# jolibrain/joliGEN

Hardware: AMD Instinct MI355X
Metric: train images/sec at 256x256 (DDPM UNet step) (higher is better)
Workload: dtype bf16; 1 GPU; palette_model DDPM, efficient UNet unet_mha ngf64 mults[1,2,4,8] res_blocks[2,2,2,2] mid-attn 16x32, 256x256, batch 32/GPU, inpainting synthetic masks, AdamW+EMA, iter_size 1 (example_ddpm_noglasses2glasses.json + SURVEY Appendix C overrides); global_batch=32, per_gpu_batch=32, image_size=256, efficient=True, parallelism=dp1, n_ranks_seen=1

## Files before the change

joligen_amd/csrc/attention.hip:

```cpp
#include "common.h"

namespace {

constexpr int D = 32;
constexpr int BQ = 128;
constexpr int BK = 128;

__device__ __forceinline__ int fsw(int row) { return (-(row >> 2)) & 3; }
__device__ __forceinline__ int bsw(int row) { return (row >> 2) & 1; }

template <typename T, int MODE>
__device__ __forceinline__ void stage_load(const T* __restrict__ g, long ld, int tid, uint4* r) {
#pragma unroll
  for (int i = 0; i < 2; ++i) {
    const int pos = i * 256 + tid, row = pos >> 2, c = pos & 3;
    r[i] = *reinterpret_cast<const uint4*>(g + (long)row * ld + c * 8);
  }
}
template <int MODE>
__device__ __forceinline__ void stage_store(uint4* lds, int tid, const uint4* r) {
#pragma unroll
  for (int i = 0; i < 2; ++i) {
    const int pos = i * 256 + tid, row = pos >> 2, c = pos & 3;
    const int pc = MODE == 0 ? (c ^ fsw(row)) : ((((c >> 1) ^ bsw(row)) << 1) | (c & 1));
    lds[row * 4 + pc] = r[i];
  }
}
__device__ __forceinline__ uint4 frag_rows(const uint4* lds, int tile, int l15, int g) {
  const int row = tile * 16 + l15;
  return lds[row * 4 + (g ^ fsw(row))];
}
__device__ __forceinline__ uint4 frag_tr(const uint4* lds, int blk, int dt, int l15, int g) {
  const char* base = reinterpret_cast<const char*>(lds);
  uint32_t w[4];
#pragma unroll
  for (int h = 0; h < 2; ++h) {
    const int row = blk * 32 + h * 16 + g * 4 + (l15 >> 2);
    const int off = row * 64 + ((dt ^ bsw(row)) << 5) + (l15 & 3) * 8;
    const uint2 u = __builtin_bit_cast(uint2, __builtin_amdgcn_ds_read_tr16_b64_v4i16((lds_v4)(base + off)));
    w[2 * h] = u.x;
    w[2 * h + 1] = u.y;
  }
  return make_uint4(w[0], w[1], w[2], w[3]);
}
template <typename T> __device__ __forceinline__ uint4 pack_p(const f32x4& a, const f32x4& b) {
  float f[8] = {a[0], a[1], a[2], a[3], b[0], b[1], b[2], b[3]};
  return pack8<T>(f);
}

struct AttnP {
  const char* qkv; char* a; float* L;
  const char* da; const char* o; char* dqkv; float* Dq;
  int B, T, nh;
  float scale;
};

template <typename T>
__global__ __launch_bounds__(256) void attn_fwd_kernel(AttnP p) {
  __shared__ uint4 sK[2][BK * 4], sV[2][BK * 4];
  const int tid = threadIdx.x, lane = tid & 63, wave = tid >> 6;
  const int l15 = lane & 15, g = lane >> 4;
  const int bh = blockIdx.y, b = bh / p.nh, h = bh % p.nh;
  const int C3 = 3 * p.nh * D;
  const T* base = (const T*)p.qkv + (long)b * p.T * C3 + h * 3 * D;
  const int q0 = blockIdx.x * BQ + wave * 32;

  uint4 fq[2];
#pragma unroll
  for (int qt = 0; qt < 2; ++qt) fq[qt] = *reinterpret_cast<const uint4*>(base + (long)(q0 + qt * 16 + l15) * C3 + g * 8);

  const int nchunk = p.T / BK;
  uint4 rk[2], rv[2];

  float mrun[2] = {-1e30f, -1e30f}, lrun[2] = {0.f, 0.f};
  stage_load<T, 0>(base + D, C3, tid, rk);
  stage_store<0>(sK[0], tid, rk);
  __syncthreads();
  for (int c = 0; c < nchunk; ++c) {
    const int cur = c & 1;
    if (c + 1 < nchunk) stage_load<T, 0>(base + (long)(c + 1) * BK * C3 + D, C3, tid, rk);
#pragma unroll
    for (int kt = 0; kt < 8; ++kt) {
      const uint4 fk = frag_rows(sK[cur], kt, l15, g);
#pragma unroll
      for (int qt = 0; qt < 2; ++qt) {
        f32x4 s = Mfma<T>::run(fk, fq[qt], (f32x4){0.f, 0.f, 0.f, 0.f});
        float mx = fmaxf(fmaxf(s[0], s[1]), fmaxf(s[2], s[3])) * p.scale;
        const float mnew = fmaxf(mrun[qt], mx);
        float acc = lrun[qt] * __expf(mrun[qt] - mnew);
#pragma unroll
        for (int r = 0; r < 4; ++r) acc += __expf(s[r] * p.scale - mnew);
        mrun[qt] = mnew;
        lrun[qt] = acc;
      }
    }
    if (c + 1 < nchunk) stage_store<0>(sK[cur ^ 1], tid, rk);
    __syncthreads();
  }
  float Lq[2];
#pragma unroll
  for (int qt = 0; qt < 2; ++qt) {
    float m = mrun[qt];
    m = fmaxf(m, __shfl_xor(m, 16));
    m = fmaxf(m, __shfl_xor(m, 32));
    float l = lrun[qt] * __expf(mrun[qt] - m);
    l += __shfl_xor(l, 16);
    l += __shfl_xor(l, 32);
    Lq[qt] = m + __logf(l);
    if (g == 0) p.L[(long)bh * p.T + q0 + qt * 16 + l15] = Lq[qt];
  }

  f32x4 o[2][2];
#pragma unroll
  for (int qt = 0; qt < 2; ++qt)
#pragma unroll
    for (int dt = 0; dt < 2; ++dt) o[qt][dt] = (f32x4){0.f, 0.f, 0.f, 0.f};
  stage_load<T, 0>(base + D, C3, tid, rk);
  stage_load<T, 1>(base + 2 * D, C3, tid, rv);
  stage_store<0>(sK[0], tid, rk);
  stage_store<1>(sV[0], tid, rv);
  __syncthreads();
  for (int c = 0; c < nchunk; ++c) {
    const int cur = c & 1;
    if (c + 1 < nchunk) {
      stage_load<T, 0>(base + (long)(c + 1) * BK * C3 + D, C3, tid, rk);
      stage_load<T, 1>(base + (long)(c + 1) * BK * C3 + 2 * D, C3, tid, rv);
    }
#pragma unroll
    for (int kb = 0; kb < 4; ++kb) {
      const uint4 fk0 = frag_rows(sK[cur], 2 * kb, l15, g), fk1 = frag_rows(sK[cur], 2 * kb + 1, l15, g);
      const uint4 fv0 = frag_tr(sV[cur], kb, 0, l15, g), fv1 = frag_tr(sV[cur], kb, 1, l15, g);
#pragma unroll
      for (int qt = 0; qt < 2; ++qt) {
        f32x4 s0 = Mfma<T>::run(fk0, fq[qt], (f32x4){0.f, 0.f, 0.f, 0.f});
        f32x4 s1 = Mfma<T>::run(fk1, fq[qt], (f32x4){0.f, 0.f, 0.f, 0.f});
#pragma unroll
        for (int r = 0; r < 4; ++r) {
          s0[r] = __expf(s0[r] * p.scale - Lq[qt]);
          s1[r] = __expf(s1[r] * p.scale - Lq[qt]);
        }
        const uint4 fp = pack_p<T>(s0, s1);
        o[qt][0] = Mfma<T>::run(fp, fv0, o[qt][0]);
        o[qt][1] = Mfma<T>::run(fp, fv1, o[qt][1]);
      }
    }
    if (c + 1 < nchunk) {
      stage_store<0>(sK[cur ^ 1], tid, rk);
      stage_store<1>(sV[cur ^ 1], tid, rv);
    }
    __syncthreads();
  }
  T* ab = (T*)p.a + (long)b * p.T * (p.nh * D) + h * D;
#pragma unroll
  for (int qt = 0; qt < 2; ++qt)
#pragma unroll
    for (int dt = 0; dt < 2; ++dt)
#pragma unroll
      for (int r = 0; r < 4; ++r)
        ab[(long)(q0 + qt * 16 + g * 4 + r) * (p.nh * D) + dt * 16 + l15] = from_f32<T>(o[qt][dt][r]);
}

template <typename T>
__global__ __launch_bounds__(256) void attn_bwd_dq_kernel(AttnP p) {
  __shared__ uint4 sK[2][BK * 4], sKt[2][BK * 4], sV[2][BK * 4];
  const int tid = threadIdx.x, lane = tid & 63, wave = tid >> 6;
  const int l15 = lane & 15, g = lane >> 4;
  const int bh = blockIdx.y, b = bh / p.nh, h = bh % p.nh;
  const int C3 = 3 * p.nh * D, C1 = p.nh * D;
  const T* base = (const T*)p.qkv + (long)b * p.T * C3 + h * 3 * D;
  const T* dab = (const T*)p.da + (long)b * p.T * C1 + h * D;
  const T* ob = (const T*)p.o + (long)b * p.T * C1 + h * D;
  const int q0 = blockIdx.x * BQ + wave * 32;

  uint4 fq[2], fdo[2];
  float Lq[2], Dq[2];
#pragma unroll
  for (int qt = 0; qt < 2; ++qt) {
    const long q = q0 + qt * 16 + l15;
    fq[qt] = *reinterpret_cast<const uint4*>(base + q * C3 + g * 8);
    fdo[qt] = *reinterpret_cast<const uint4*>(dab + q * C1 + g * 8);
    const uint4 fo = *reinterpret_cast<const uint4*>(ob + q * C1 + g * 8);
    float a[8], c[8];
    unpack8<T>(fdo[qt], a);
    unpack8<T>(fo, c);
    float d = 0.f;
#pragma unroll
    for (int i = 0; i < 8; ++i) d += a[i] * c[i];
    d += __shfl_xor(d, 16);
    d += __shfl_xor(d, 32);
    Dq[qt] = d;
    Lq[qt] = p.L[(long)bh * p.T + q];
    if (g == 0) p.Dq[(long)bh * p.T + q] = d;
  }
  f32x4 dq[2][2];
#pragma unroll
  for (int qt = 0; qt < 2; ++qt)
#pragma unroll
    for (int dt = 0; dt < 2; ++dt) dq[qt][dt] = (f32x4){0.f, 0.f, 0.f, 0.f};

  const int nchunk = p.T / BK;
  uint4 rk[2], rv[2];
  stage_load<T, 0>(base + D, C3, tid, rk);
  stage_load<T, 0>(base + 2 * D, C3, tid, rv);
  stage_store<0>(sK[0], tid, rk);
  stage_store<1>(sKt[0], tid, rk);
  stage_store<0>(sV[0], tid, rv);
  __syncthreads();
  for (int c = 0; c < nchunk; ++c) {
    const int cur = c & 1;
    if (c + 1 < nchunk) {
      stage_load<T, 0>(base + (long)(c + 1) * BK * C3 + D, C3, tid, rk);
      stage_load<T, 0>(base + (long)(c + 1) * BK * C3 + 2 * D, C3, tid, rv);
    }
#pragma unroll
    for (int kb = 0; kb < 4; ++kb) {
      const uint4 fk0 = frag_rows(sK[cur], 2 * kb, l15, g), fk1 = frag_rows(sK[cur], 2 * kb + 1, l15, g);
      const uint4 fv0 = frag_rows(sV[cur], 2 * kb, l15, g), fv1 = frag_rows(sV[cur], 2 * kb + 1, l15, g);
      const uint4 fkt0 = frag_tr(sKt[cur], kb, 0, l15, g), fkt1 = frag_tr(sKt[cur], kb, 1, l15, g);
#pragma unroll
      for (int qt = 0; qt < 2; ++qt) {
        const f32x4 z = {0.f, 0.f, 0.f, 0.f};
        f32x4 s0 = Mfma<T>::run(fk0, fq[qt], z), s1 = Mfma<T>::run(fk1, fq[qt], z);
        f32x4 d0 = Mfma<T>::run(fv0, fdo[qt], z), d1 = Mfma<T>::run(fv1, fdo[qt], z);
#pragma unroll
        for (int r = 0; r < 4; ++r) {
          s0[r] = __expf(s0[r] * p.scale - Lq[qt]) * (d0[r] - Dq[qt]);
          s1[r] = __expf(s1[r] * p.scale - Lq[qt]) * (d1[r] - Dq[qt]);
        }
        const uint4 fds = pack_p<T>(s0, s1);
        dq[qt][0] = Mfma<T>::run(fds, fkt0, dq[qt][0]);
        dq[qt][1] = Mfma<T>::run(fds, fkt1, dq[qt][1]);
      }
    }
    if (c + 1 < nchunk) {
      stage_store<0>(sK[cur ^ 1], tid, rk);
      stage_store<1>(sKt[cur ^ 1], tid, rk);
      stage_store<0>(sV[cur ^ 1], tid, rv);
    }
    __syncthreads();
  }
  T* dqb = (T*)p.dqkv + (long)b * p.T * C3 + h * 3 * D;
#pragma unroll
  for (int qt = 0; qt < 2; ++qt)
#pragma unroll
    for (int dt = 0; dt < 2; ++dt)
#pragma unroll
      for (int r = 0; r < 4; ++r)
        dqb[(long)(q0 + qt * 16 + g * 4 + r) * C3 + dt * 16 + l15] = from_f32<T>(dq[qt][dt][r] * p.scale);
}

template <typename T>
__global__ __launch_bounds__(256) void attn_bwd_dkv_kernel(AttnP p) {
  __shared__ uint4 sQ[2][BK * 4], sQt[2][BK * 4], sO[2][BK * 4], sOt[2][BK * 4];
  __shared__ float sL[2][BK], sD[2][BK];
  const int tid = threadIdx.x, lane = tid & 63, wave = tid >> 6;
  const int l15 = lane & 15, g = lane >> 4;
  const int bh = blockIdx.y, b = bh / p.nh, h = bh % p.nh;
  const int C3 = 3 * p.nh * D, C1 = p.nh * D;
  const T* base = (const T*)p.qkv + (long)b * p.T * C3 + h * 3 * D;
  const T* dab = (const T*)p.da + (long)b * p.T * C1 + h * D;
  const int k0 = blockIdx.x * BQ + wave * 32;

  uint4 fk[2], fv[2];
#pragma unroll
  for (int kt = 0; kt < 2; ++kt) {
    fk[kt] = *reinterpret_cast<const uint4*>(base + (long)(k0 + kt * 16 + l15) * C3 + D + g * 8);
    fv[kt] = *reinterpret_cast<const uint4*>(base + (long)(k0 + kt * 16 + l15) * C3 + 2 * D + g * 8);
  }
  f32x4 dk[2][2], dv[2][2];
#pragma unroll
  for (int kt = 0; kt < 2; ++kt)
#pragma unroll
    for (int dt = 0; dt < 2; ++dt) dk[kt][dt] = dv[kt][dt] = (f32x4){0.f, 0.f, 0.f, 0.f};

  const int nchunk = p.T / BK;
  uint4 rq[2], ro[2];
  float rl = 0.f, rd = 0.f;
  auto load = [&](int c) {
    stage_load<T, 0>(base + (long)c * BK * C3, C3, tid, rq);
    stage_load<T, 0>(dab + (long)c * BK * C1, C1, tid, ro);
    if (tid < BK) {
      rl = p.L[(long)bh * p.T + c * BK + tid];
      rd = p.Dq[(long)bh * p.T + c * BK + tid];
    }
  };
  auto store = [&](int buf) {
    stage_store<0>(sQ[buf], tid, rq);
    stage_store<1>(sQt[buf], tid, rq);
    stage_store<0>(sO[buf], tid, ro);
    stage_store<1>(sOt[buf], tid, ro);
    if (tid < BK) {
      sL[buf][tid] = rl;
      sD[buf][tid] = rd;
    }
  };
  load(0);
  store(0);
  __syncthreads();
  for (int c = 0; c < nchunk; ++c) {
    const int cur = c & 1;
    if (c + 1 < nchunk) load(c + 1);
#pragma unroll
    for (int qb = 0; qb < 4; ++qb) {
      const uint4 fq0 = frag_rows(sQ[cur], 2 * qb, l15, g), fq1 = frag_rows(sQ[cur], 2 * qb + 1, l15, g);
      const uint4 fo0 = frag_rows(sO[cur], 2 * qb, l15, g), fo1 = frag_rows(sO[cur], 2 * qb + 1, l15, g);
      const uint4 fqt0 = frag_tr(sQt[cur], qb, 0, l15, g), fqt1 = frag_tr(sQt[cur], qb, 1, l15, g);
      const uint4 fot0 = frag_tr(sOt[cur], qb, 0, l15, g), fot1 = frag_tr(sOt[cur], qb, 1, l15, g);
      const float4 L0 = *reinterpret_cast<const float4*>(&sL[cur][qb * 32 + g * 4]);
      const float4 L1 = *reinterpret_cast<const float4*>(&sL[cur][qb * 32 + 16 + g * 4]);
      const float4 D0 = *reinterpret_cast<const float4*>(&sD[cur][qb * 32 + g * 4]);
      const float4 D1 = *reinterpret_cast<const float4*>(&sD[cur][qb * 32 + 16 + g * 4]);
      const float l0[4] = {L0.x, L0.y, L0.z, L0.w}, l1[4] = {L1.x, L1.y, L1.z, L1.w};
      const float e0[4] = {D0.x, D0.y, D0.z, D0.w}, e1[4] = {D1.x, D1.y, D1.z, D1.w};
#pragma unroll
      for (int kt = 0; kt < 2; ++kt) {
        const f32x4 z = {0.f, 0.f, 0.f, 0.f};
        f32x4 s0 = Mfma<T>::run(fq0, fk[kt], z), s1 = Mfma<T>::run(fq1, fk[kt], z);
        f32x4 d0 = Mfma<T>::run(fo0, fv[kt], z), d1 = Mfma<T>::run(fo1, fv[kt], z);
        f32x4 ds0, ds1;
#pragma unroll
        for (int r = 0; r < 4; ++r) {
          s0[r] = __expf(s0[r] * p.scale - l0[r]);
          s1[r] = __expf(s1[r] * p.scale - l1[r]);
          ds0[r] = s0[r] * (d0[r] - e0[r]);
          ds1[r] = s1[r] * (d1[r] - e1[r]);
        }
        const uint4 fp = pack_p<T>(s0, s1), fds = pack_p<T>(ds0, ds1);
        dv[kt][0] = Mfma<T>::run(fp, fot0, dv[kt][0]);
        dv[kt][1] = Mfma<T>::run(fp, fot1, dv[kt][1]);
        dk[kt][0] = Mfma<T>::run(fds, fqt0, dk[kt][0]);
        dk[kt][1] = Mfma<T>::run(fds, fqt1, dk[kt][1]);
      }
    }
    if (c + 1 < nchunk) store(cur ^ 1);
    __syncthreads();
  }
  T* dqb = (T*)p.dqkv + (long)b * p.T * C3 + h * 3 * D;
#pragma unroll
  for (int kt = 0; kt < 2; ++kt)
#pragma unroll
    for (int dt = 0; dt < 2; ++dt)
#pragma unroll
      for (int r = 0; r < 4; ++r) {
        const long row = (long)(k0 + kt * 16 + g * 4 + r) * C3 + dt * 16 + l15;
        dqb[row + D] = from_f32<T>(dk[kt][dt][r] * p.scale);
        dqb[row + 2 * D] = from_f32<T>(dv[kt][dt][r]);
      }
}

}

extern "C" int jg_attention_fwd(int dtype, const void* qkv, void* a, float* L, int B, int T, int heads, int head_dim,
                                jg_stream_t s) {
  if (!qkv || !a || !L || B < 1 || heads < 1) return JG_ERR_BAD_ARG;
  if (head_dim != D || T % BQ) return JG_ERR_UNSUPPORTED;
  AttnP p = {};
  p.qkv = (const char*)qkv; p.a = (char*)a; p.L = L; p.B = B; p.T = T; p.nh = heads;
  p.scale = 1.0f / sqrtf((float)head_dim);
  dim3 grid(T / BQ, B * heads);
  JG_DISPATCH_DTYPE(dtype, hipLaunchKernelGGL((attn_fwd_kernel<T>), grid, dim3(256), 0, (hipStream_t)s, p););
  JG_CHECK_LAUNCH();
  return JG_OK;
}

extern "C" int jg_attention_bwd(int dtype, const void* qkv, const void* o, const float* L, const void* da, void* dqkv,
                                float* Dq, int B, int T, int heads, int head_dim, jg_stream_t s) {
  if (!qkv || !o || !L || !da || !dqkv || !Dq || B < 1 || heads < 1) return JG_ERR_BAD_ARG;
  if (head_dim != D || T % BQ) return JG_ERR_UNSUPPORTED;
  AttnP p = {};
  p.qkv = (const char*)qkv; p.o = (const char*)o; p.L = const_cast<float*>(L); p.da = (const char*)da;
  p.dqkv = (char*)dqkv; p.Dq = Dq; p.B = B; p.T = T; p.nh = heads;
  p.scale = 1.0f / sqrtf((float)head_dim);
  dim3 grid(T / BQ, B * heads);
  JG_DISPATCH_DTYPE(dtype, hipLaunchKernelGGL((attn_bwd_dq_kernel<T>), grid, dim3(256), 0, (hipStream_t)s, p);
                    hipLaunchKernelGGL((attn_bwd_dkv_kernel<T>), grid, dim3(256), 0, (hipStream_t)s, p););
  JG_CHECK_LAUNCH();
  return JG_OK;
}
```

joligen_amd/csrc/common.h:

```cpp
#pragma once
#include <hip/hip_runtime.h>
#include <stdint.h>

#include "../../include/jg355.h"

typedef _Float16 f16_t;
typedef __bf16 bf16_t;
typedef _Float16 f16x8 __attribute__((ext_vector_type(8)));
typedef __bf16 bf16x8 __attribute__((ext_vector_type(8)));
typedef float f32x4 __attribute__((ext_vector_type(4)));
typedef short s16x4_t __attribute__((ext_vector_type(4)));
typedef __attribute__((address_space(3))) s16x4_t* lds_v4;

#define JG_WAVE 64

#define JG_TUNE_LIST(X) \
  X(HALO_CFG, 0) X(WGRAD_HALO_CFG, 0) X(CONV_VARIANT, 6) X(WGRAD_VARIANT, 4) X(SINKHORN_GENERIC, 0) X(CONV1X1, 1) X(GN_REVERSE, 1) \
  X(HALO_DBG, 0) X(PERSIST64, 1) X(HALO_PIPE, 1) X(WGRAD_PIPE, 1) X(CONV_SPLITK, 1) X(CONV_SMALL_TILE, 1) X(GN_FUSED, 1)           \
  X(GN_FUSED_CAP, 256) X(GN_FUSED_DBG, 0) X(GN_FUSED_SLEEP, 4) X(WGRAD_LDS_PAD, 0) X(LN_BWD_CAP, 256) X(DW_BWD_CAP, 512)           \
  X(DW_BWD_PPT, 8) X(CONV_KXK, 1) X(CONV_RING, 1) X(WGRAD_DEEP, 1) X(WGRAD_SW, 0) X(DETERMINISTIC, 0) X(WGRAD_GROUP_BLOCKS, 1024)  \
  X(SGEMM_SPLIT, 0) X(WGRAD_BIG, 1) X(DW_RUN, 1) X(SUBPIXEL_DGRAD_CFG, 0)
#define JG_TUNE_ENUM(name, dflt) JG_TUNE_##name,
enum JgTune { JG_TUNE_LIST(JG_TUNE_ENUM) JG_TUNE_COUNT };
#undef JG_TUNE_ENUM
int jg_tune(int which);
void jg_note_kernel(const char* name);

#define JG_CHECK_LAUNCH()                          \
  do {                                             \
    if (hipGetLastError() != hipSuccess) return JG_ERR_LAUNCH; \
  } while (0)

template <typename T> __device__ __forceinline__ float to_f32(T v) { return (float)v; }
template <typename T> __device__ __forceinline__ T from_f32(float v) { return (T)v; }

template <typename T> __device__ __forceinline__ T bits_to(uint16_t b) { return __builtin_bit_cast(T, b); }
template <typename T> __device__ __forceinline__ uint16_t to_bits(T v) { return __builtin_bit_cast(uint16_t, v); }

template <typename T> __device__ __forceinline__ void unpack8(const uint4& v, float* f) {
  const uint32_t w[4] = {v.x, v.y, v.z, v.w};
#pragma unroll
  for (int i = 0; i < 4; ++i) {
    f[2 * i] = to_f32(bits_to<T>((uint16_t)(w[i] & 0xffffu)));
    f[2 * i + 1] = to_f32(bits_to<T>((uint16_t)(w[i] >> 16)));
  }
}
template <typename T> __device__ __forceinline__ uint4 pack8(const float* f) {
  uint32_t w[4];
#pragma unroll
  for (int i = 0; i < 4; ++i) {
    w[i] = (uint32_t)to_bits<T>(from_f32<T>(f[2 * i])) | ((uint32_t)to_bits<T>(from_f32<T>(f[2 * i + 1])) << 16);
  }
  return make_uint4(w[0], w[1], w[2], w[3]);
}
template <typename T> __device__ __forceinline__ uint2 pack4(float a, float b, float c, float d) {
  uint2 r;
  r.x = (uint32_t)to_bits<T>(from_f32<T>(a)) | ((uint32_t)to_bits<T>(from_f32<T>(b)) << 16);
  r.y = (uint32_t)to_bits<T>(from_f32<T>(c)) | ((uint32_t)to_bits<T>(from_f32<T>(d)) << 16);
  return r;
}
template <typename T> __device__ __forceinline__ void unpack4(const uint2& v, float* f) {
  f[0] = to_f32(bits_to<T>((uint16_t)(v.x & 0xffffu)));
  f[1] = to_f32(bits_to<T>((uint16_t)(v.x >> 16)));
  f[2] = to_f32(bits_to<T>((uint16_t)(v.y & 0xffffu)));
  f[3] = to_f32(bits_to<T>((uint16_t)(v.y >> 16)));
}

template <typename T> struct Mfma;
template <> struct Mfma<f16_t> {
  static __device__ __forceinline__ f32x4 run(const uint4& a, const uint4& b, f32x4 c) {
    return __builtin_amdgcn_mfma_f32_16x16x32_f16(__builtin_bit_cast(f16x8, a), __builtin_bit_cast(f16x8, b), c, 0, 0, 0);
  }
};
template <> struct Mfma<bf16_t> {
  static __device__ __forceinline__ f32x4 run(const uint4& a, const uint4& b, f32x4 c) {
    return __builtin_amdgcn_mfma_f32_16x16x32_bf16(__builtin_bit_cast(bf16x8, a), __builtin_bit_cast(bf16x8, b), c, 0, 0, 0);
  }
};

template <typename T> __device__ __forceinline__ uint4 ldg16(const T* ptr, bool ok) {
  uint4 v = *reinterpret_cast<const uint4*>(ptr);
  v.x = ok ? v.x : 0u;
  v.y = ok ? v.y : 0u;
  v.z = ok ? v.z : 0u;
  v.w = ok ? v.w : 0u;
  return v;
}

__device__ __forceinline__ float sigmoid_fast(float u) { return __builtin_amdgcn_rcpf(1.0f + __expf(-u)); }
__device__ __forceinline__ float silu_f(float u) { return u * sigmoid_fast(u); }
__device__ __forceinline__ float silu_grad_f(float u) {
  const float s = sigmoid_fast(u);
  return s * (1.0f + u * (1.0f - s));
}

template <int ACT> __device__ __forceinline__ float act_f(float u) {
  if (ACT == JG_ACT_SILU) return silu_f(u);
  if (ACT == JG_ACT_RELU) return fmaxf(u, 0.f);
  if (ACT == JG_ACT_LRELU) return u > 0.f ? u : 0.2f * u;
  return u;
}
template <int ACT> __device__ __forceinline__ float act_grad_f(float u) {
  if (ACT == JG_ACT_SILU) return silu_grad_f(u);
  if (ACT == JG_ACT_RELU) return u > 0.f ? 1.f : 0.f;
  if (ACT == JG_ACT_LRELU) return u > 0.f ? 1.f : 0.2f;
  return 1.f;
}
__device__ __forceinline__ float act_grad_rt(float u, int act) {
  return act == JG_ACT_SILU ? silu_grad_f(u) : act == JG_ACT_RELU ? (u > 0.f ? 1.f : 0.f) : act == JG_ACT_LRELU ? (u > 0.f ? 1.f : 0.2f) : 1.f;
}

#define JG_DISPATCH_ACT(act, ...)                          \
  do {                                                     \
    if ((act) == JG_ACT_SILU) { constexpr int ACT = JG_ACT_SILU; __VA_ARGS__ }        \
    else if ((act) == JG_ACT_RELU) { constexpr int ACT = JG_ACT_RELU; __VA_ARGS__ }   \
    else if ((act) == JG_ACT_LRELU) { constexpr int ACT = JG_ACT_LRELU; __VA_ARGS__ } \
    else { constexpr int ACT = JG_ACT_NONE; __VA_ARGS__ }                              \
  } while (0)

__device__ __forceinline__ float wave_sum(float v) {
#pragma unroll
  for (int o = 32; o > 0; o >>= 1) v += __shfl_xor(v, o);
  return v;
}
__device__ __forceinline__ float wave_max(float v) {
#pragma unroll
  for (int o = 32; o > 0; o >>= 1) v = fmaxf(v, __shfl_xor(v, o));
  return v;
}

#define JG_DISPATCH_DTYPE(dtype, ...)                 \
  do {                                                \
    if ((dtype) == JG_F16) {                          \
      typedef f16_t T;                                \
      __VA_ARGS__                                     \
    } else if ((dtype) == JG_BF16) {                  \
      typedef bf16_t T;                               \
      __VA_ARGS__                                     \
    } else {                                          \
      return JG_ERR_BAD_ARG;                          \
    }                                                 \
  } while (0)
```

Before: 659.8 images/sec.

## Add one-pass flash attention forward with LDS DMA staging and exp2 softmax

After: 664.9 images/sec (median of 6 runs). No clear change (+0.8%).

```diff
diff --git a/joligen_amd/csrc/attention.hip b/joligen_amd/csrc/attention.hip
--- a/joligen_amd/csrc/attention.hip
+++ b/joligen_amd/csrc/attention.hip
@@ -1,4 +1,4 @@
-#include "common.h"
+#include "lds_dma.h"
 
 namespace {
 
@@ -24,6 +24,24 @@
     const int pos = i * 256 + tid, row = pos >> 2, c = pos & 3;
     const int pc = MODE == 0 ? (c ^ fsw(row)) : ((((c >> 1) ^ bsw(row)) << 1) | (c & 1));
     lds[row * 4 + pc] = r[i];
+  }
+}
+typedef uint32_t u32x4 __attribute__((ext_vector_type(4)));
+struct Staged { u32x4 c0, c1; };
+template <typename T, int MODE>
+__device__ __forceinline__ void stage_load(const T* __restrict__ g, long ld, int tid, Staged& r) {
+  const int row = tid >> 2, c = tid & 3;
+  r.c0 = *reinterpret_cast<const u32x4*>(g + (long)row * ld + c * 8);
+  r.c1 = *reinterpret_cast<const u32x4*>(g + (long)(row + 64) * ld + c * 8);
+}
+template <int MODE>
+__device__ __forceinline__ void stage_store(uint4* lds, int tid, const Staged& r) {
+  const int c = tid & 3;
+#pragma unroll
+  for (int i = 0; i < 2; ++i) {
+    const int row = i * 64 + (tid >> 2);
+    const int pc = MODE == 0 ? (c ^ fsw(row)) : ((((c >> 1) ^ bsw(row)) << 1) | (c & 1));
+    *reinterpret_cast<u32x4*>(&lds[row * 4 + pc]) = i == 0 ? r.c0 : r.c1;
   }
 }
 __device__ __forceinline__ uint4 frag_rows(const uint4* lds, int tile, int l15, int g) {
@@ -43,6 +61,14 @@
   }
   return make_uint4(w[0], w[1], w[2], w[3]);
 }
+template <typename T, int MODE>
+__device__ __forceinline__ void stage_dma(const T* __restrict__ g, long ld, int tid, int wave, unsigned lds_tile) {
+  const int row = tid >> 2, pc = tid & 3;
+  const int c = MODE == 0 ? (pc ^ fsw(row)) : ((((pc >> 1) ^ bsw(row)) << 1) | (pc & 1));
+  glds16(g + (long)row * ld + c * 8, lds_tile + wave * 1024);
+  glds16(g + (long)(row + 64) * ld + c * 8, lds_tile + 4096 + wave * 1024);
+}
+__device__ __forceinline__ void landed(uint4& v) { asm volatile("" : "+v"(v.x), "+v"(v.y), "+v"(v.z), "+v"(v.w)); }
 template <typename T> __device__ __forceinline__ uint4 pack_p(const f32x4& a, const f32x4& b) {
   float f[8] = {a[0], a[1], a[2], a[3], b[0], b[1], b[2], b[3]};
   return pack8<T>(f);
@@ -55,8 +81,113 @@
   float scale;
 };
 
+constexpr float LOG2E = 1.4426950408889634f, LN2 = 0.6931471805599453f;
+__device__ __forceinline__ float exp2_fast(float x) { return __builtin_amdgcn_exp2f(x); }
+
+__device__ __forceinline__ float max4(float m, const f32x4& s) { return fmaxf(fmaxf(m, fmaxf(s[0], s[1])), fmaxf(s[2], s[3])); }
+
 template <typename T>
-__global__ __launch_bounds__(256) void attn_fwd_kernel(AttnP p) {
+__global__ __launch_bounds__(256, 4) void attn_fwd_kernel(AttnP p) {
+  __shared__ uint4 sK[2][BK * 4], sV[2][BK * 4];
+  const int tid = threadIdx.x, lane = tid & 63, wave = __builtin_amdgcn_readfirstlane(tid >> 6);
+  const int l15 = lane & 15, g = lane >> 4;
+  const int bh = blockIdx.y, b = bh / p.nh, h = bh % p.nh;
+  const int C3 = 3 * p.nh * D;
+  const T* base = (const T*)p.qkv + (long)b * p.T * C3 + h * 3 * D;
+  const int q0 = blockIdx.x * BQ + wave * 32;
+  const float c2 = p.scale * LOG2E;
+  typedef __attribute__((address_space(3))) char* lds_cptr;
+  const unsigned ldsK = (unsigned)(size_t)(lds_cptr)(char*)&sK[0][0], ldsV = (unsigned)(size_t)(lds_cptr)(char*)&sV[0][0];
+
+  uint4 fq[2];
+#pragma unroll
+  for (int qt = 0; qt < 2; ++qt) fq[qt] = *reinterpret_cast<const uint4*>(base + (long)(q0 + qt * 16 + l15) * C3 + g * 8);
+
+  float mrun[2] = {-1e30f, -1e30f}, lrun[2] = {0.f, 0.f};
+  f32x4 o[2][2];
+#pragma unroll
+  for (int qt = 0; qt < 2; ++qt)
+#pragma unroll
+    for (int dt = 0; dt < 2; ++dt) o[qt][dt] = (f32x4){0.f, 0.f, 0.f, 0.f};
+
+  const int nchunk = p.T / BK;
+  stage_dma<T, 0>(base + D, C3, tid, wave, ldsK);
+  stage_dma<T, 1>(base + 2 * D, C3, tid, wave, ldsV);
+  landed(fq[0]);
+  landed(fq[1]);
+  wait_vmcnt<0>();
+  __syncthreads();
+  for (int c = 0; c < nchunk; ++c) {
+    const int cur = c & 1;
+    if (c + 1 < nchunk) {
+      stage_dma<T, 0>(base + (long)(c + 1) * BK * C3 + D, C3, tid, wave, ldsK + (cur ^ 1) * (BK * 64));
+      stage_dma<T, 1>(base + (long)(c + 1) * BK * C3 + 2 * D, C3, tid, wave, ldsV + (cur ^ 1) * (BK * 64));
+    }
+    f32x4 s[8][2];
+#pragma unroll
+    for (int kt = 0; kt < 8; ++kt) {
+      const uint4 fk = frag_rows(sK[cur], kt, l15, g);
+#pragma unroll
+      for (int qt = 0; qt < 2; ++qt) s[kt][qt] = Mfma<T>::run(fk, fq[qt], (f32x4){0.f, 0.f, 0.f, 0.f});
+    }
+#pragma unroll
+    for (int qt = 0; qt < 2; ++qt) {
+      float mx = -1e30f;
+#pragma unroll
+      for (int kt = 0; kt < 8; ++kt) mx = max4(mx, s[kt][qt]);
+      mx = fmaxf(mx, __shfl_xor(mx, 16));
+      mx = fmaxf(mx, __shfl_xor(mx, 32));
+      const float mnew = fmaxf(mrun[qt], mx * c2);
+      const float alpha = exp2_fast(mrun[qt] - mnew);
+      mrun[qt] = mnew;
+      lrun[qt] *= alpha;
+#pragma unroll
+      for (int r = 0; r < 4; ++r) {
+        const float ar = __shfl(alpha, g * 4 + r);
+        o[qt][0][r] *= ar;
+        o[qt][1][r] *= ar;
+      }
+    }
+#pragma unroll
+    for (int kb = 0; kb < 4; ++kb) {
+      const uint4 fv0 = frag_tr(sV[cur], kb, 0, l15, g), fv1 = frag_tr(sV[cur], kb, 1, l15, g);
+#pragma unroll
+      for (int qt = 0; qt < 2; ++qt) {
+        f32x4 p0, p1;
+#pragma unroll
+        for (int r = 0; r < 4; ++r) {
+          p0[r] = exp2_fast(fmaf(s[2 * kb][qt][r], c2, -mrun[qt]));
+          p1[r] = exp2_fast(fmaf(s[2 * kb + 1][qt][r], c2, -mrun[qt]));
+        }
+        lrun[qt] += ((p0[0] + p0[1]) + (p0[2] + p0[3])) + ((p1[0] + p1[1]) + (p1[2] + p1[3]));
+        const uint4 fp = pack_p<T>(p0, p1);
+        o[qt][0] = Mfma<T>::run(fp, fv0, o[qt][0]);
+        o[qt][1] = Mfma<T>::run(fp, fv1, o[qt][1]);
+      }
+    }
+    wait_vmcnt<0>();
+    __syncthreads();
+  }
+  T* ab = (T*)p.a + (long)b * p.T * (p.nh * D) + h * D;
+#pragma unroll
+  for (int qt = 0; qt < 2; ++qt) {
+    float l = lrun[qt];
+    l += __shfl_xor(l, 16);
+    l += __shfl_xor(l, 32);
+    if (g == 0) p.L[(long)bh * p.T + q0 + qt * 16 + l15] = mrun[qt] * LN2 + __logf(l);
+    const float inv = 1.0f / l;
+#pragma unroll
+    for (int r = 0; r < 4; ++r) {
+      const float ir = __shfl(inv, g * 4 + r);
+#pragma unroll
+      for (int dt = 0; dt < 2; ++dt)
+        ab[(long)(q0 + qt * 16 + g * 4 + r) * (p.nh * D) + dt * 16 + l15] = from_f32<T>(o[qt][dt][r] * ir);
+    }
+  }
+}
+
+template <typename T>
+__global__ __launch_bounds__(256) void attn_fwd_twopass_kernel(AttnP p) {
   __shared__ uint4 sK[2][BK * 4], sV[2][BK * 4];
   const int tid = threadIdx.x, lane = tid & 63, wave = tid >> 6;
   const int l15 = lane & 15, g = lane >> 4;
@@ -161,7 +292,7 @@
 }
 
 template <typename T>
-__global__ __launch_bounds__(256) void attn_bwd_dq_kernel(AttnP p) {
+__global__ __launch_bounds__(256, 2) void attn_bwd_dq_kernel(AttnP p) {
   __shared__ uint4 sK[2][BK * 4], sKt[2][BK * 4], sV[2][BK * 4];
   const int tid = threadIdx.x, lane = tid & 63, wave = tid >> 6;
   const int l15 = lane & 15, g = lane >> 4;
@@ -171,6 +302,7 @@
   const T* dab = (const T*)p.da + (long)b * p.T * C1 + h * D;
   const T* ob = (const T*)p.o + (long)b * p.T * C1 + h * D;
   const int q0 = blockIdx.x * BQ + wave * 32;
+  const float c2 = p.scale * LOG2E;
 
   uint4 fq[2], fdo[2];
   float Lq[2], Dq[2];
@@ -189,7 +321,7 @@
     d += __shfl_xor(d, 16);
     d += __shfl_xor(d, 32);
     Dq[qt] = d;
-    Lq[qt] = p.L[(long)bh * p.T + q];
+    Lq[qt] = p.L[(long)bh * p.T + q] * LOG2E;
     if (g == 0) p.Dq[(long)bh * p.T + q] = d;
   }
   f32x4 dq[2][2];
@@ -199,7 +331,7 @@
     for (int dt = 0; dt < 2; ++dt) dq[qt][dt] = (f32x4){0.f, 0.f, 0.f, 0.f};
 
   const int nchunk = p.T / BK;
-  uint4 rk[2], rv[2];
+  Staged rk, rv;
   stage_load<T, 0>(base + D, C3, tid, rk);
   stage_load<T, 0>(base + 2 * D, C3, tid, rv);
   stage_store<0>(sK[0], tid, rk);
@@ -224,8 +356,8 @@
         f32x4 d0 = Mfma<T>::run(fv0, fdo[qt], z), d1 = Mfma<T>::run(fv1, fdo[qt], z);
 #pragma unroll
         for (int r = 0; r < 4; ++r) {
-          s0[r] = __expf(s0[r] * p.scale - Lq[qt]) * (d0[r] - Dq[qt]);
-          s1[r] = __expf(s1[r] * p.scale - Lq[qt]) * (d1[r] - Dq[qt]);
+          s0[r] = exp2_fast(fmaf(s0[r], c2, -Lq[qt])) * (d0[r] - Dq[qt]);
+          s1[r] = exp2_fast(fmaf(s1[r], c2, -Lq[qt])) * (d1[r] - Dq[qt]);
         }
         const uint4 fds = pack_p<T>(s0, s1);
         dq[qt][0] = Mfma<T>::run(fds, fkt0, dq[qt][0]);
@@ -250,7 +382,7 @@
 }
 
 template <typename T>
-__global__ __launch_bounds__(256) void attn_bwd_dkv_kernel(AttnP p) {
+__global__ __launch_bounds__(256, 2) void attn_bwd_dkv_kernel(AttnP p) {
   __shared__ uint4 sQ[2][BK * 4], sQt[2][BK * 4], sO[2][BK * 4], sOt[2][BK * 4];
   __shared__ float sL[2][BK], sD[2][BK];
   const int tid = threadIdx.x, lane = tid & 63, wave = tid >> 6;
@@ -260,6 +392,7 @@
   const T* base = (const T*)p.qkv + (long)b * p.T * C3 + h * 3 * D;
   const T* dab = (const T*)p.da + (long)b * p.T * C1 + h * D;
   const int k0 = blockIdx.x * BQ + wave * 32;
+  const float c2 = p.scale * LOG2E;
 
   uint4 fk[2], fv[2];
 #pragma unroll
@@ -274,13 +407,13 @@
     for (int dt = 0; dt < 2; ++dt) dk[kt][dt] = dv[kt][dt] = (f32x4){0.f, 0.f, 0.f, 0.f};
 
   const int nchunk = p.T / BK;
-  uint4 rq[2], ro[2];
+  Staged rq, ro;
   float rl = 0.f, rd = 0.f;
   auto load = [&](int c) {
     stage_load<T, 0>(base + (long)c * BK * C3, C3, tid, rq);
     stage_load<T, 0>(dab + (long)c * BK * C1, C1, tid, ro);
     if (tid < BK) {
-      rl = p.L[(long)bh * p.T + c * BK + tid];
+      rl = p.L[(long)bh * p.T + c * BK + tid] * LOG2E;
       rd = p.Dq[(long)bh * p.T + c * BK + tid];
     }
   };
@@ -320,8 +453,8 @@
         f32x4 ds0, ds1;
 #pragma unroll
         for (int r = 0; r < 4; ++r) {
-          s0[r] = __expf(s0[r] * p.scale - l0[r]);
-          s1[r] = __expf(s1[r] * p.scale - l1[r]);
+          s0[r] = exp2_fast(fmaf(s0[r], c2, -l0[r]));
+          s1[r] = exp2_fast(fmaf(s1[r], c2, -l1[r]));
           ds0[r] = s0[r] * (d0[r] - e0[r]);
           ds1[r] = s1[r] * (d1[r] - e1[r]);
         }
@@ -358,7 +491,11 @@
   p.qkv = (const char*)qkv; p.a = (char*)a; p.L = L; p.B = B; p.T = T; p.nh = heads;
   p.scale = 1.0f / sqrtf((float)head_dim);
   dim3 grid(T / BQ, B * heads);
-  JG_DISPATCH_DTYPE(dtype, hipLaunchKernelGGL((attn_fwd_kernel<T>), grid, dim3(256), 0, (hipStream_t)s, p););
+  if (jg_tune(JG_TUNE_ATTN_ONEPASS) != 0) {
+    JG_DISPATCH_DTYPE(dtype, hipLaunchKernelGGL((attn_fwd_kernel<T>), grid, dim3(256), 0, (hipStream_t)s, p););
+  } else {
+    JG_DISPATCH_DTYPE(dtype, hipLaunchKernelGGL((attn_fwd_twopass_kernel<T>), grid, dim3(256), 0, (hipStream_t)s, p););
+  }
   JG_CHECK_LAUNCH();
   return JG_OK;
 }
diff --git a/joligen_amd/csrc/common.h b/joligen_amd/csrc/common.h
--- a/joligen_amd/csrc/common.h
+++ b/joligen_amd/csrc/common.h
@@ -19,7 +19,7 @@
   X(HALO_DBG, 0) X(PERSIST64, 1) X(HALO_PIPE, 1) X(WGRAD_PIPE, 1) X(CONV_SPLITK, 1) X(CONV_SMALL_TILE, 1) X(GN_FUSED, 1)           \
   X(GN_FUSED_CAP, 256) X(GN_FUSED_DBG, 0) X(GN_FUSED_SLEEP, 4) X(WGRAD_LDS_PAD, 0) X(LN_BWD_CAP, 256) X(DW_BWD_CAP, 512)           \
   X(DW_BWD_PPT, 8) X(CONV_KXK, 1) X(CONV_RING, 1) X(WGRAD_DEEP, 1) X(WGRAD_SW, 0) X(DETERMINISTIC, 0) X(WGRAD_GROUP_BLOCKS, 1024)  \
-  X(SGEMM_SPLIT, 0) X(WGRAD_BIG, 1) X(DW_RUN, 1) X(SUBPIXEL_DGRAD_CFG, 0)
+  X(SGEMM_SPLIT, 0) X(WGRAD_BIG, 1) X(DW_RUN, 1) X(SUBPIXEL_DGRAD_CFG, 0) X(ATTN_ONEPASS, 1)
 #define JG_TUNE_ENUM(name, dflt) JG_TUNE_##name,
 enum JgTune { JG_TUNE_LIST(JG_TUNE_ENUM) JG_TUNE_COUNT };
 #undef JG_TUNE_ENUM
```
